# sauloal/pykmer

Measured on AMD Instinct MI355X. Metric: bp/s k-mer counted (k=15, 1 GPU), higher is better.
Workload: dtype u8; 1 GPU; k=15 canonical k-mer count of one 800 Mbp synthetic genome per GPU (SURVEY 8d C2, seed 2+rank), 4^15 table resident in HBM; fasta_bytes=813333854, num_kmers=766212116, parallelism=1 independent genome(s)

## Files before the change

include/pykmer_hip.h:

```cpp
#ifndef PYKMER_HIP_H
#define PYKMER_HIP_H

#include <stddef.h>
#include <stdint.h>

#ifdef __cplusplus
extern "C" {
#endif

#define PK_ABI_VERSION 3

enum {
    PK_OK = 0,
    PK_ERR_ARG = -1,
    PK_ERR_HIP = -2,
    PK_ERR_RECS_CAP = -3,
    PK_ERR_STATE = -4,
    PK_ERR_FORMAT = -5
};

#define PK_FORMAT_FASTA 0
#define PK_FORMAT_FASTQ 1

typedef struct pk_record {
// ... 122 lines not shown
       PK_CORR_FIELDS = 6 };
typedef struct pk_correct pk_correct;
int pk_correct_create(pk_correct **out, int k, int device);
int pk_correct_set_tables(pk_correct *c, const void *const *dev_tables, int N, int min_count, int max_count);
int pk_correct_set_cover(pk_correct *c, const uint8_t *cover, uint64_t n_bases, int min_qual_byte, int min_windows);
int pk_correct_feed(pk_correct *c, const uint8_t *host_text, uint64_t n_bytes, const uint64_t *starts, uint64_t n_records,
                    uint8_t *host_text_out, uint64_t *out);
int pk_correct_feed_device(pk_correct *c, const void *dev_text, uint64_t n_bytes, const uint64_t *starts, uint64_t n_records,
                           void *dev_text_out, uint64_t *out);
int pk_correct_finish(pk_correct *c, uint64_t totals_out[6]);
int pk_correct_timings(pk_correct *c, double out[2]);
void pk_correct_destroy(pk_correct *c);

typedef struct pk_unitig pk_unitig;
int pk_unitig_create(pk_unitig **out, int k, int device);
int pk_unitig_build(pk_unitig *u, const void *dev_table, int min_count, int max_count, uint64_t min_kmers, uint64_t totals_out[8]);
int pk_unitig_rows(pk_unitig *u, uint64_t *first_addr, uint64_t *n_kmers, uint64_t *depth, uint8_t *circular, uint64_t cap);
int pk_unitig_text(pk_unitig *u, uint8_t *host_out, uint64_t offset, uint64_t n_bytes);
int pk_unitig_timings(pk_unitig *u, double out[4]);
void pk_unitig_destroy(pk_unitig *u);

int pk_bgzf_scan(const uint8_t *src, uint64_t n_bytes, uint64_t cap, uint64_t *c_off_out, uint64_t *c_size_out,
                 uint64_t *isize_out, uint64_t *n_blocks_out);
int pk_bgzf_inflate(const uint8_t *src, uint64_t src_bytes, const uint64_t *c_off, const uint64_t *c_size,
                    const uint64_t *u_off, uint64_t n_blocks, uint8_t *dst, int threads);
int pk_bgzf_deflate(const uint8_t *src, uint64_t n_bytes, int level, uint32_t block_input, uint8_t *dst, uint64_t dst_cap,
                    uint64_t *c_sizes_out, uint64_t *total_out, int threads);

int pk_diag_occupancy(int which);
int pk_diag_plan(int k, uint64_t n_bytes, uint64_t out[8]);
int pk_diag_settled_chunks(pk_indexer *ix, uint64_t *out);
int pk_diag_plan_slice(int k, int n_slices, uint64_t n_bytes, uint64_t out[16]);
int pk_diag_level2_order(const uint32_t *sizes, uint32_t B1, uint32_t *order_out);

#ifdef __cplusplus
}
#endif
#endif
```

pykmer_amd/_lib.py:

```python
import ctypes
import os

import numpy as np

_HERE = os.path.dirname(os.path.abspath(__file__))
from ._rt import LIB_PATH, open_library

PK_OK, PK_ERR_ARG, PK_ERR_HIP, PK_ERR_RECS_CAP, PK_ERR_STATE, PK_ERR_FORMAT = 0, -1, -2, -3, -4, -5
PK_FORMAT_FASTA, PK_FORMAT_FASTQ = 0, 1
FORMATS = {"fasta": PK_FORMAT_FASTA, "fastq": PK_FORMAT_FASTQ}
MASK_HARD, MASK_INVERT = 1, 2

RECORD_DTYPE = np.dtype([("name_off", "<u8"), ("name_len", "<u8"), ("seq_len", "<u8"), ("n_valid_kmers", "<u8")])

_u64p = ctypes.POINTER(ctypes.c_uint64)
_SIGNATURES = {
    "pk_version": (ctypes.c_int, []),
    "pk_last_error": (ctypes.c_int, [ctypes.c_char_p, ctypes.c_size_t]),
    "pk_device_count": (ctypes.c_int, []),
    "pk_warm": (ctypes.c_int, [ctypes.c_int]),
    "pk_dev_alloc": (ctypes.c_int, [ctypes.POINTER(ctypes.c_void_p), ctypes.c_uint64, ctypes.c_int]),
    "pk_dev_free": (ctypes.c_int, [ctypes.c_void_p, ctypes.c_int]),
    "pk_dev_upload": (ctypes.c_int, [ctypes.c_void_p, ctypes.c_void_p, ctypes.c_uint64, ctypes.c_int]),
    "pk_dev_download": (ctypes.c_int, [ctypes.c_void_p, ctypes.c_void_p, ctypes.c_uint64, ctypes.c_int]),
# ... 72 lines not shown
    "pk_trim_create": (ctypes.c_int, [ctypes.POINTER(ctypes.c_void_p), ctypes.c_int]),
    "pk_trim_set_cover": (ctypes.c_int, [ctypes.c_void_p, ctypes.c_void_p, ctypes.c_uint64, ctypes.c_int]),
    "pk_trim_feed": (ctypes.c_int, [ctypes.c_void_p, ctypes.c_void_p, ctypes.c_uint64, ctypes.c_void_p, ctypes.c_uint64, ctypes.c_void_p]),
    "pk_trim_feed_device": (ctypes.c_int, [ctypes.c_void_p, ctypes.c_void_p, ctypes.c_uint64, ctypes.c_void_p, ctypes.c_uint64, ctypes.c_void_p]),
    "pk_trim_finish": (ctypes.c_int, [ctypes.c_void_p, ctypes.c_void_p]),
    "pk_trim_timings": (ctypes.c_int, [ctypes.c_void_p, ctypes.c_void_p]),
    "pk_trim_destroy": (None, [ctypes.c_void_p]),
    "pk_correct_create": (ctypes.c_int, [ctypes.POINTER(ctypes.c_void_p), ctypes.c_int, ctypes.c_int]),
    "pk_correct_set_tables": (ctypes.c_int, [ctypes.c_void_p, ctypes.c_void_p, ctypes.c_int, ctypes.c_int, ctypes.c_int]),
    "pk_correct_set_cover": (ctypes.c_int, [ctypes.c_void_p, ctypes.c_void_p, ctypes.c_uint64, ctypes.c_int, ctypes.c_int]),
    "pk_correct_feed": (ctypes.c_int, [ctypes.c_void_p, ctypes.c_void_p, ctypes.c_uint64, ctypes.c_void_p, ctypes.c_uint64, ctypes.c_void_p,
                                        ctypes.c_void_p]),
    "pk_correct_feed_device": (ctypes.c_int, [ctypes.c_void_p, ctypes.c_void_p, ctypes.c_uint64, ctypes.c_void_p, ctypes.c_uint64, ctypes.c_void_p,
                                               ctypes.c_void_p]),
    "pk_correct_finish": (ctypes.c_int, [ctypes.c_void_p, ctypes.c_void_p]),
    "pk_correct_timings": (ctypes.c_int, [ctypes.c_void_p, ctypes.c_void_p]),
    "pk_correct_destroy": (None, [ctypes.c_void_p]),
    "pk_unitig_create": (ctypes.c_int, [ctypes.POINTER(ctypes.c_void_p), ctypes.c_int, ctypes.c_int]),
    "pk_unitig_build": (ctypes.c_int, [ctypes.c_void_p, ctypes.c_void_p, ctypes.c_int, ctypes.c_int, ctypes.c_uint64, ctypes.c_void_p]),
    "pk_unitig_rows": (ctypes.c_int, [ctypes.c_void_p, ctypes.c_void_p, ctypes.c_void_p, ctypes.c_void_p, ctypes.c_void_p, ctypes.c_uint64]),
    "pk_unitig_text": (ctypes.c_int, [ctypes.c_void_p, ctypes.c_void_p, ctypes.c_uint64, ctypes.c_uint64]),
    "pk_unitig_timings": (ctypes.c_int, [ctypes.c_void_p, ctypes.c_void_p]),
    "pk_unitig_destroy": (None, [ctypes.c_void_p]),
    "pk_bgzf_scan": (ctypes.c_int, [ctypes.c_void_p, ctypes.c_uint64, ctypes.c_uint64, ctypes.c_void_p, ctypes.c_void_p, ctypes.c_void_p, _u64p]),
    "pk_bgzf_inflate": (ctypes.c_int, [ctypes.c_void_p, ctypes.c_uint64, ctypes.c_void_p, ctypes.c_void_p, ctypes.c_void_p, ctypes.c_uint64, ctypes.c_void_p,
                                        ctypes.c_int]),
    "pk_bgzf_deflate": (ctypes.c_int, [ctypes.c_void_p, ctypes.c_uint64, ctypes.c_int, ctypes.c_uint32, ctypes.c_void_p, ctypes.c_uint64,
                                        ctypes.c_void_p, _u64p, ctypes.c_int]),
    "pk_diag_occupancy": (ctypes.c_int, [ctypes.c_int]),
    "pk_diag_plan": (ctypes.c_int, [ctypes.c_int, ctypes.c_uint64, ctypes.c_void_p]),
    "pk_diag_settled_chunks": (ctypes.c_int, [ctypes.c_void_p, _u64p]),
    "pk_diag_plan_slice": (ctypes.c_int, [ctypes.c_int, ctypes.c_int, ctypes.c_uint64, ctypes.c_void_p]),
    "pk_diag_level2_order": (ctypes.c_int, [ctypes.c_void_p, ctypes.c_uint32, ctypes.c_void_p]),
}
EXPORTS = tuple(_SIGNATURES)

_lib = None


class PkError(RuntimeError):
    def __init__(self, code, message):
        super().__init__(f"libpykmer_hip error {code}: {message}")
        self.code = code


def load():
    global _lib
    if _lib is None:
        lib = open_library()
        for name, (res, args) in _SIGNATURES.items():
            fn = getattr(lib, name)
            fn.restype, fn.argtypes = res, args
        _lib = lib
    return _lib


def _check(rc):
    if rc != PK_OK:
        buf = ctypes.create_string_buffer(512)
        load().pk_last_error(buf, 512)
        msg = buf.value.decode("utf-8", "replace")
        if rc == PK_ERR_ARG:
            raise ValueError(msg)
        raise PkError(rc, msg)


# ... 689 lines not shown

def bgzf_deflate(data: np.ndarray, level: int, block_input: int, threads: int):
    n_blocks = (data.size + block_input - 1) // block_input
    dst = np.empty(max(1, n_blocks) * 65536, dtype=np.uint8)
    sizes = np.zeros(max(1, n_blocks), dtype=np.uint64)
    total = ctypes.c_uint64(0)
    _check(load().pk_bgzf_deflate(data.ctypes.data, data.size, level, block_input, dst.ctypes.data, dst.size, sizes.ctypes.data,
                                  ctypes.byref(total), int(threads)))
    return dst[: total.value], sizes[:n_blocks].astype(np.int64)


def diag_plan(k: int, n_bytes: int = 0) -> dict:
    out = np.zeros(8, dtype=np.uint64)
    _check(load().pk_diag_plan(k, n_bytes, out.ctypes.data))
    names = ("feed_max", "capacity1", "capacity2", "B1", "B2", "fb_bits", "n_chunks", "fits_u32")
    return {n: int(v) for n, v in zip(names, out)}


WS_VARIANTS = ("narrow", "narrow_sliced", "k15", "k17", "wide_sliced", "deep", "wide")
COUNT_KERNELS = ("whole", "bytes", "half")


def diag_plan_slice(k: int, n_slices: int = 1, n_bytes: int = 0) -> dict:
    out = np.zeros(16, dtype=np.uint64)
    _check(load().pk_diag_plan_slice(k, n_slices, n_bytes, out.ctypes.data))
    names = ("addr_bits", "fb_bits", "b1", "b2", "sample_stride", "n_tally", "sample2", "n_chunks", "variant", "count_kernel",
             "split", "B1", "B2", "capacity1", "capacity2", "fits_u32")
    d = {n: int(v) for n, v in zip(names, out)}
    d["variant"] = WS_VARIANTS[d["variant"]]
    d["count_kernel"] = COUNT_KERNELS[d["count_kernel"]]
    return d


def diag_level2_order(sizes) -> np.ndarray:
    s = np.ascontiguousarray(sizes, dtype=np.uint32)
    out = np.zeros(max(1, s.size), dtype=np.uint32)
    _check(load().pk_diag_level2_order(s.ctypes.data, s.size, out.ctypes.data))
    return out[:s.size]


def gram_expand(pair: np.ndarray) -> np.ndarray:
    p = np.ascontiguousarray(pair, dtype=np.uint64)
    N = p.shape[0]
    m = np.zeros((N, N, 3), dtype=np.uint64)
    _check(load().pk_gram_expand(p.ctypes.data, N, m.ctypes.data))
    return m
```

pykmer_amd/csrc/kmer_part.hip:

```cpp
#include <cstddef>
#include <string>
#include <type_traits>
#include "../../include/pykmer_hip.h"
#include "part_common.h"

namespace pk {

int set_error(int code, const std::string &msg);

__global__ __launch_bounds__(1024) void k_sample2(const uint32_t *__restrict__ in, const uint32_t *__restrict__ bucket_base,
                                                  const uint32_t *__restrict__ bucket_end, PartPlan pl, uint32_t stride2,
                                                  uint32_t *__restrict__ tally, uint32_t *__restrict__ sampled_n,
                                                  const uint32_t *__restrict__ flags) {
    __shared__ uint32_t h[512];
    __shared__ uint32_t n_seen;
    if (flags[0]) return;
    const uint32_t b = blockIdx.x, lo = bucket_base[b], hi = bucket_end[b];
    if (threadIdx.x < 512) h[threadIdx.x] = 0;
    if (threadIdx.x == 0) n_seen = 0;
    __syncthreads();
    const uint32_t n_grp = (hi - lo + 255u) / 256u, n_sgrp = (n_grp + stride2 - 1u) / stride2;
    const uint32_t mask = pl.B2 - 1u, shift = pl.fb_bits, w = threadIdx.x >> 6, lane = threadIdx.x & 63u;
    uint32_t mine = 0;
    for (uint32_t s0 = 0; s0 < n_sgrp; s0 += 8u * 16u) {
// ... 138 lines not shown
            }
            const bool full = v_lo == win && n_tile == (uint32_t)TILE;
            uint32_t okm = 0;
            if (!full) {
#pragma unroll
                for (int j = 0; j < PER / 4; j++) {
                    const uint32_t i = win + (threadIdx.x + j * NT) * 4u;
#pragma unroll
                    for (int e = 0; e < 4; e++) okm |= (i + e >= v_lo && i + e < v_hi) ? (1u << (j * 4 + e)) : 0u;
                }
            }
            if (win + TILE < hi) fetch(win + TILE, nxt);
            uint32_t *cl = cursor + (uint64_t)b * B;
            const uint32_t *ce = cap_end + (uint64_t)b * B;
            if (full) scatter_tile<uint32_t, false, NT, PER, 512, true, 8, REC24>(L, r, 0u, n_tile, shift, B, low_mask, true, out, settle, cl, ce, dump, flags);
            else scatter_tile<uint32_t, false, NT, PER, 512, false, 8, REC24>(L, r, okm, n_tile, shift, B, low_mask, true, out, settle, cl, ce, dump, flags);
        }
    };
    const uint32_t *pos = wg2_start;
    const uint32_t per = pl.B1 >> 3;
    const uint32_t o_lo = (blockIdx.x & 7u) * per, o_hi = o_lo + per, first = blockIdx.x >> 3, step = gridDim.x >> 3;
    const uint32_t w_end = pos[o_hi];
    for (uint32_t w = pos[o_lo] + first; w < w_end; w += step) {
        uint32_t a = o_lo, z = o_hi;
        while (z - a > 1) { const uint32_t m = (a + z) >> 1; if (pos[m] <= w) a = m; else z = m; }
        const uint32_t b = l2_order[a];
        const uint64_t s = (uint64_t)bucket_base[b] + (uint64_t)(w - pos[a]) * pl.R2;
        const uint64_t e = min(s + pl.R2, (uint64_t)bucket_end[b]);
        item(b, (uint32_t)s, (uint32_t)e);
    }
}

constexpr uint32_t K6_PIECE = 65024;
constexpr int K6_BYTES_LDS = 65536 + 1024 + 128;

__device__ __forceinline__ int wave_sum_i32(int v) {
    v += __builtin_amdgcn_update_dpp(0, v, 0x128, 0xf, 0xf, false);
    v += __builtin_amdgcn_update_dpp(0, v, 0x124, 0xf, 0xf, false);
    v += __builtin_amdgcn_update_dpp(0, v, 0x122, 0xf, 0xf, false);
    v += __builtin_amdgcn_update_dpp(0, v, 0x121, 0xf, 0xf, false);
    return __builtin_amdgcn_readlane(v, 0) + __builtin_amdgcn_readlane(v, 16) + __builtin_amdgcn_readlane(v, 32) +
           __builtin_amdgcn_readlane(v, 48);
}

typedef unsigned short U16x2 __attribute__((ext_vector_type(2)));
__device__ __forceinline__ uint32_t clamp255_pair(uint32_t x) {
    const U16x2 lim = {255, 255};
    return __builtin_bit_cast(uint32_t, __builtin_elementwise_min(__builtin_bit_cast(U16x2, x), lim));
}
__device__ __forceinline__ uint32_t pack_low_bytes(uint32_t x0, uint32_t x1) {
    return __builtin_amdgcn_perm(x1, x0, 0x06040200u);
}

struct SliceTally {
    int d1 = 0, d2 = 0;
    __device__ __forceinline__ void add_dword(int *dh, uint32_t x, int sign) {
        uint32_t p0 = x & 0x01010101u, p1 = (x >> 1) & 0x01010101u;
        uint32_t rest = p0 & p1;
        const uint32_t high = x & 0xfcfcfcfcu;
        if (high) {
            const uint32_t big = (((high & 0x7f7f7f7fu) + 0x7f7f7f7fu) | high) & 0x80808080u;
            const uint32_t keep = ~(big >> 7);
            p0 &= keep; p1 &= keep;
            rest = (p0 & p1) | (big >> 7);
        }
        const int n1 = (int)__builtin_popcount(p0 & ~p1), n2 = (int)__builtin_popcount(p1 & ~p0);
        d1 += sign * n1; d2 += sign * n2;
        while (rest) {
            const int bit = __ffs(rest) - 1;
            atomicAdd(&dh[(x >> bit) & 0xffu], sign);
            rest &= rest - 1u;
        }
    }
};

template <int T, bool LEAN, bool NOREC = false>
__device__ __forceinline__ void bucket_count_body(const uint16_t *__restrict__ recs, const uint32_t *__restrict__ final_start,
                                                  const uint32_t *__restrict__ final_end, uint32_t fb_bits, uint32_t split_bits,
                                                  uint8_t *__restrict__ table8, uint32_t fresh, unsigned long long *__restrict__ hist_rep, uint8_t *smem,
                                                  int *dh, uint32_t wg) {
    uint32_t *cnt = reinterpret_cast<uint32_t *>(smem);
    const uint32_t fb = wg >> split_bits, part = wg & ((1u << split_bits) - 1u);
    const uint32_t start = final_start[fb], end = final_end ? final_end[fb] : final_start[fb + 1];
    const uint32_t part_bits = fb_bits - split_bits;
    const uint32_t n_addr = 1u << part_bits;
    uint8_t *slice = table8 + ((uint64_t)fb << fb_bits) + (uint64_t)part * n_addr;
    if (start == end) {
        if (fresh) {
            if (n_addr >= 16) for (uint32_t g = threadIdx.x; g < n_addr / 16; g += T) reinterpret_cast<uint4 *>(slice)[g] = make_uint4(0, 0, 0, 0);
            else for (uint32_t a = threadIdx.x; a < n_addr; a += T) slice[a] = 0;
        }
        return;
    }
    const uint32_t base = start & ~7u;
    const uint32_t i_first = base + threadIdx.x * 8;
    uint4 v_first = make_uint4(0, 0, 0, 0);
    if (i_first < min(base + K6_PIECE, end)) v_first = *reinterpret_cast<const uint4 *>(recs + i_first);
    const bool by_rec = NOREC ? false : (((end - start) >> split_bits) < n_addr / 4 || n_addr < 16);
    SliceTally tally;
    for (uint32_t i = threadIdx.x; i < 256; i += T) dh[i] = 0;
    if (fresh) {
        if (n_addr >= 8) for (uint32_t g = threadIdx.x; g < n_addr / 8; g += T) reinterpret_cast<uint4 *>(cnt)[g] = make_uint4(0, 0, 0, 0);
        else for (uint32_t a = threadIdx.x; a < max(n_addr / 2, 1u); a += T) cnt[a] = 0u;
    } else if (n_addr >= 16) {
        if (!by_rec) __syncthreads();
        for (uint32_t g = threadIdx.x; g < n_addr / 16; g += T) {
            uint4 v = reinterpret_cast<const uint4 *>(slice)[g];
            uint32_t w[4] = {v.x, v.y, v.z, v.w};
            if (!by_rec) {
#pragma unroll
                for (int q = 0; q < 4; q++) tally.add_dword(dh, w[q], -1);
            }
#pragma unroll
            for (int q = 0; q < 8; q++)
                cnt[g * 8 + q] = __builtin_amdgcn_perm(0u, w[q >> 1], (q & 1) ? 0x0c030c02u : 0x0c010c00u);
        }
    } else {
        for (uint32_t a = threadIdx.x; a < max(n_addr / 2, 1u); a += T) cnt[a] = slice[2 * a] | (n_addr > 1u ? (uint32_t)slice[2 * a + 1] << 16 : 0u);
    }
    __syncthreads();
    auto bump = [&](uint32_t a, uint32_t n) {
        const uint32_t sh = 16u * (a & 1u);
        if (!by_rec) { atomicAdd(&cnt[a >> 1], n << sh); return; }
        int &d1 = tally.d1, &d2 = tally.d2;
        const uint32_t c = (atomicAdd(&cnt[a >> 1], n << sh) >> sh) & 0xffffu;
        const uint32_t oc = c > 255u ? 255u : c, nc = c + n > 255u ? 255u : c + n;
        if (oc == nc) return;
        if (nc == 1u) d1++;
        else if (nc == 2u && oc == 1u) { d2++; d1--; }
        else {
            atomicAdd(&dh[nc], 1);
// ... 91 lines not shown
                for (int q = 0; q < 4; q++) tally.add_dword(dh, o[q], 1);
            }
            reinterpret_cast<uint4 *>(slice)[g] = make_uint4(o[0], o[1], o[2], o[3]);
        }
    } else {
        for (uint32_t a = threadIdx.x; a < max(n_addr / 2, 1u); a += T) {
            uint32_t x = cnt[a], lo = x & 0xffffu, hi = x >> 16;
            slice[2 * a] = (uint8_t)(lo > 255u ? 255u : lo);
            if (n_addr > 1u) slice[2 * a + 1] = (uint8_t)(hi > 255u ? 255u : hi);
        }
    }
    const int d1 = wave_sum_i32(tally.d1), d2 = wave_sum_i32(tally.d2);
    if ((threadIdx.x & 63) == 0) {
        if (d1) atomicAdd(&dh[1], d1);
        if (d2) atomicAdd(&dh[2], d2);
    }
    __syncthreads();
    for (uint32_t i = threadIdx.x; i < 256; i += T) {
        const int v = dh[i];
        if (v) atomicAdd(&hist_rep[(uint64_t)(blockIdx.x % HIST_REPLICAS) * 256 + i], (unsigned long long)(long long)v);
    }
}

template <int T>
__global__ __launch_bounds__(T) void k_bucket_count(const uint16_t *__restrict__ recs, const uint32_t *__restrict__ final_start,
                                                    const uint32_t *__restrict__ final_end, uint32_t fb_bits, uint32_t split_bits,
                                                    uint8_t *__restrict__ table8, uint32_t fresh, unsigned long long *__restrict__ hist_rep,
                                                    const uint32_t *__restrict__ flags) {
    extern __shared__ __attribute__((aligned(16))) uint8_t smem[];
    __shared__ int dh[256];
    if (flags[0]) return;
    bucket_count_body<T, true>(recs, final_start, final_end, fb_bits, split_bits, table8, fresh, hist_rep, smem, dh, blockIdx.x);
}
template <int T, bool FRESH>
__global__ __launch_bounds__(T) __attribute__((amdgpu_waves_per_eu(8, 8)))
void k_bucket_count_half_lean(const uint16_t *__restrict__ recs, const uint32_t *__restrict__ final_start, const uint32_t *__restrict__ final_end,
                              uint32_t fb_bits, uint32_t split_bits, uint8_t *__restrict__ table8, uint32_t fresh, unsigned long long *__restrict__ hist_rep,
                              const uint32_t *__restrict__ flags) {
    extern __shared__ __attribute__((aligned(16))) uint8_t smem[];
    __shared__ int dh[256];
    if (flags[0]) return;
    bucket_count_body<T, true, true>(recs, final_start, final_end, 15u, 0u, table8, FRESH ? 1u : 0u, hist_rep, smem, dh, blockIdx.x);
}

template <int T>
__global__ __launch_bounds__(T) __attribute__((amdgpu_waves_per_eu(8, 8)))
void k_bucket_count_bytes(const uint16_t *__restrict__ recs, const uint32_t *__restrict__ final_start, const uint32_t *__restrict__ final_end,
                          uint8_t *__restrict__ table8, uint32_t fresh, unsigned long long *__restrict__ hist_rep,
                          const uint32_t *__restrict__ flags) {
    extern __shared__ __attribute__((aligned(128))) uint8_t smem[];
    constexpr uint32_t N_ADDR = 65536u;
    int *dh = reinterpret_cast<int *>(smem + N_ADDR);
    uint32_t *wrap_flag = reinterpret_cast<uint32_t *>(smem + N_ADDR + 1024);
    if (flags[0]) return;
    const uint32_t fb = blockIdx.x;
    const uint32_t start = final_start[fb], end = final_end ? final_end[fb] : final_start[fb + 1];
    uint4 *slice = reinterpret_cast<uint4 *>(table8 + ((uint64_t)fb << 16));
    uint4 *img = reinterpret_cast<uint4 *>(smem);
    if (start == end) {
        if (fresh) for (uint32_t g = threadIdx.x; g < N_ADDR / 16; g += T) slice[g] = make_uint4(0, 0, 0, 0);
        return;
    }
    bool recount = end - start >= 16384u;
    int d1 = 0, d2 = 0;
    if (!recount) {
        const uint32_t base = start & ~7u;
        const uint32_t i_first = base + threadIdx.x * 8;
        uint4 v = make_uint4(0, 0, 0, 0);
        if (i_first < end) v = *reinterpret_cast<const uint4 *>(recs + i_first);
        for (uint32_t i = threadIdx.x; i < 256; i += T) dh[i] = 0;
        if (threadIdx.x == 0) *wrap_flag = 0u;
        if (fresh) { for (uint32_t g = threadIdx.x; g < N_ADDR / 16; g += T) img[g] = make_uint4(0, 0, 0, 0); }
        else { for (uint32_t g = threadIdx.x; g < N_ADDR / 16; g += T) img[g] = slice[g]; }
        __syncthreads();
        uint32_t *cnt = reinterpret_cast<uint32_t *>(smem);
// ... 145 lines not shown
    pl.n_wg1 = pl.n_chunks < wg1 ? pl.n_chunks : wg1;
    if (pl.n_wg1 == 0) pl.n_wg1 = 1;
    pl.G1 = (pl.n_chunks + pl.n_wg1 - 1) / pl.n_wg1;
    if (pl.G1 == 0) pl.G1 = 1;
    pl.R2 = 4u * TILE;
    pl.sample_stride = pl.n_chunks >= 1024u ? 16u : 1u;
    const uint64_t nfb = (uint64_t)pl.B1 * pl.B2;
    pl.n_tally = (pl.b2 && nfb <= 32768 && pl.addr_bits <= 30) ? (uint32_t)nfb : pl.B1;
    pl.sample2 = (pl.b2 && pl.n_tally == pl.B1 && nfb <= 262144 && pl.B1 >= 8u) ? 1u : 0u;
    const uint64_t est1 = (uint64_t)pl.n_chunks * TILE + pl.B1, est2 = (uint64_t)pl.n_chunks * TILE + nfb;
    pl.capacity1 = est1 + est1 / 8 + (uint64_t)pl.B1 * 4100;
    pl.capacity2 = pl.sample2 ? est2 + est2 / 4 + nfb * 4104 : est2 + est2 / 8 + nfb * 2056;
    return pl;
}

uint32_t bucket_split(const PartPlan &pl, uint64_t n_bytes) {
    return pl.fb_bits == 16 && n_bytes / ((uint64_t)pl.B1 * pl.B2) < 8192u ? 1u : 0u;
}
CountKernel bucket_count_kernel(const PartPlan &pl, uint64_t n_bytes) {
    if (pl.fb_bits == 15) return COUNT_HALF;
    return bucket_split(pl, n_bytes) ? COUNT_BYTES : COUNT_WHOLE;
}

int part_plan_check(const PartPlan &pl, uint64_t n_bytes) {
    const auto no = [](const std::string &what) { return set_error(PK_ERR_HIP, "partition plan outside the kernels' limits: " + what); };
    const uint32_t max_B1 = pl.k <= 15 ? 128u : PART_MAX_B1;
    if (pl.B1 > max_B1 || pl.B2 > 512u || pl.fb_bits > 16u)
        return no(std::to_string(pl.B1) + " x " + std::to_string(pl.B2) + " buckets of 2^" + std::to_string(pl.fb_bits) + " addresses; the LDS arrays hold " +
                  std::to_string(max_B1) + " x 512 of 2^16");
    if (pl.b2 && pl.n_tally == pl.B1 && !pl.sample2) return no("two levels, but neither the sampling launch nor sample2 lays out the final buckets");
    if (pl.k <= 15 && pl.b2 && pl.addr_bits - pl.b1 > 24u)
        return no(std::to_string(pl.addr_bits - pl.b1) + " address bits behind the level-1 digit; its 3-byte records hold 24");
    if (bucket_split(pl, n_bytes) > 1u) return no("the bucket count is laid out for whole and half buckets");
    return PK_OK;
}

size_t part_workspace(const PartPlan &pl, uint64_t n_bytes, uint8_t *base, PartBuffers *view, PartSignals *signals) {
    PartBuffers unused, &b = view ? *view : unused;
    const size_t nfb = (size_t)pl.B1 * pl.B2, rec1 = (size_t)(pl.capacity1 + TILE + 64);
    size_t o = 0;
    const auto place = [&](auto *&p, size_t bytes, bool packed = false) {
        p = reinterpret_cast<std::remove_reference_t<decltype(p)>>(reinterpret_cast<uintptr_t>(base) + o);
        o += bytes;
        if (!packed) o = (o + 255) & ~(size_t)255;
    };
    place(b.codes, (size_t)pl.n_chunks * SLOT_CODE_WORDS * 4);
    place(b.restarts, (size_t)pl.n_chunks * SLOT_RST_WORDS * 4);
    place(b.n_bases, (size_t)pl.n_chunks * 4);
    place(b.tally_rows, (size_t)COUNT_WGS * pl.n_tally * 4);
    const bool s2 = pl.sample2 != 0;
    place(b.tally_tot, (s2 ? nfb : pl.n_tally) * 4, s2);
    place(b.sampled_n, s2 ? (size_t)pl.B1 * 4 : 0, true);
    place(b.block_tot, s2 ? 1024 * 4 : 0);
    if (!s2) b.sampled_n = b.block_tot = nullptr;
    for (uint32_t **p : {&b.bucket_base, &b.bucket_end, &b.cursor1, &b.cap_end, &b.wg2_start}) place(*p, (size_t)(pl.B1 + 1) * 4);
    place(b.l2_order, (size_t)pl.B1 * 4);
    for (uint32_t **p : {&b.final_start, &b.cursor2, &b.cap2_end}) place(*p, (nfb + 1) * 4);
    place(b.out1, !pl.b2 ? rec1 * 2 : pl.k <= 15 ? level1_hi_plane_offset(pl.capacity1) + rec1 : rec1 * 4);
    place(b.out2, !pl.b2 ? 256 : (size_t)(pl.capacity2 + TILE + 64) * 2);
    b.side_cap = n_bytes + 16;
    place(b.side, (size_t)b.side_cap * 8);
    b.signals = signals;
    b.side_n = &b.signals->side_n;
    b.flags = b.signals->flags;
    return o;
}

void part_set_attributes() {
    fuse_set_attributes();
    hipFuncSetAttribute((const void *)k_scatter2<512, 32>, hipFuncAttributeMaxDynamicSharedMemorySize, (int)SCATTER_LDS_NARROW);
    hipFuncSetAttribute((const void *)k_scatter2<512, 32, true>, hipFuncAttributeMaxDynamicSharedMemorySize, (int)SCATTER_LDS_NARROW);
    hipFuncSetAttribute((const void *)k_bucket_count<1024>, hipFuncAttributeMaxDynamicSharedMemorySize, 128 * 1024);
    hipFuncSetAttribute((const void *)k_bucket_count_half_lean<1024, true>, hipFuncAttributeMaxDynamicSharedMemorySize, 128 * 1024);
    hipFuncSetAttribute((const void *)k_bucket_count_half_lean<1024, false>, hipFuncAttributeMaxDynamicSharedMemorySize, 128 * 1024);
    hipFuncSetAttribute((const void *)k_bucket_count_bytes<1024>, hipFuncAttributeMaxDynamicSharedMemorySize, K6_BYTES_LDS);
}

extern "C" int pk_diag_occupancy(int which) {
    int n = -1;
    hipError_t e = hipErrorInvalidValue;
    if (which == 0) e = hipOccupancyMaxActiveBlocksPerMultiprocessor(&n, (const void *)k_bucket_count<1024>, 1024, 128 * 1024);
    if (which == 1) e = hipOccupancyMaxActiveBlocksPerMultiprocessor(&n, (const void *)k_bucket_count_bytes<1024>, 1024, K6_BYTES_LDS);
    if (which == 2) e = hipOccupancyMaxActiveBlocksPerMultiprocessor(&n, (const void *)k_bucket_count_half_lean<1024, true>, 1024, 65536);
    if (which == 3) e = hipOccupancyMaxActiveBlocksPerMultiprocessor(&n, (const void *)k_scatter2<512, 32>, 512, SCATTER_LDS_NARROW);
    return e == hipSuccess ? n : -(int)e;
}

extern "C" int pk_diag_level2_order(const uint32_t *sizes, uint32_t B1, uint32_t *order_out) {
    if (!sizes || !order_out) return set_error(PK_ERR_ARG, "pk_diag_level2_order: null argument");
    static_assert(PART_MAX_B1 == 512, "the message below and include/pykmer_hip.h name the limit");
    if (B1 < 8u || B1 > PART_MAX_B1 || (B1 & 7u)) return set_error(PK_ERR_ARG, "pk_diag_level2_order: B1 must be a multiple of 8 from 8 to 512");
    for (uint32_t b = 0; b < B1; b++) order_out[level2_position(level2_rank(sizes, B1, b), B1)] = b;
    return PK_OK;
}

int launch_partitioned(const PartPlan &pl, const PartBuffers &b, const L2 *st2, uint64_t n_bytes, uint32_t stride, const Carry *carry, uint8_t *table8,
                       unsigned long long *hist, unsigned long long *hist_rep, bool fresh, const PartEvents &ev, hipStream_t s) {
    const uint32_t nfb = pl.B1 * pl.B2;
    const uint32_t *flags = b.flags;
    const char *failed = nullptr;
    hipError_t why = hipSuccess;
    const auto stage = [&](const char *name) { if (!failed && (why = hipGetLastError()) != hipSuccess) failed = name; };
    launch_provision(pl, b, st2, stride, carry, s);
    stage("bucket layout");
    hipEventRecord(ev.sort_begin, s);
    launch_walk_sort(pl, b, st2, carry, s);
    stage("level-1 sort");
    hipEventRecord(ev.sort_end, s);
    const uint16_t *final_recs = (const uint16_t *)b.out1;
    const uint32_t *k6_start = b.bucket_base, *k6_end = b.bucket_end;
    if (pl.sample2) {
        const uint32_t stride2 = stride == 1u ? 1u : 16u, n_blocks = (nfb + 1023u) / 1024u;
        const uint32_t *base1 = b.bucket_base, *end1 = b.bucket_end;
        hipLaunchKernelGGL(k_sample2, dim3(pl.B1), dim3(1024), 0, s, (const uint32_t *)b.out1, base1, end1, pl, stride2, b.tally_tot, b.sampled_n, flags);
        hipLaunchKernelGGL(k_rooms2, dim3(n_blocks), dim3(1024), 0, s, (const uint32_t *)b.tally_tot, (const uint32_t *)b.sampled_n, base1, end1, pl, stride2,
                           nfb, b.final_start, b.cap2_end, b.block_tot, flags);
        hipLaunchKernelGGL(k_bases2, dim3(1), dim3(1024), 0, s, n_blocks, nfb, pl, b.block_tot, b.final_start, b.flags);
        hipLaunchKernelGGL(k_starts2, dim3(n_blocks), dim3(1024), 0, s, nfb, (const uint32_t *)b.block_tot, b.final_start, b.cursor2, b.cap2_end, flags);
        stage("final-bucket rooms");
    }
    if (pl.b2) {
        const uint32_t grid2 = 4096u;
        hipLaunchKernelGGL((pl.k <= 15 ? &k_scatter2<512, 32, true> : &k_scatter2<512, 32>), dim3(grid2), dim3(512), SCATTER_LDS_NARROW, s,
                           (const uint32_t *)b.out1, b.wg2_start, (const uint32_t *)b.l2_order, b.bucket_base, b.bucket_end, pl, b.out2, b.cursor2, (const uint32_t *)b.cap2_end,
                           (uint32_t)pl.capacity2, b.flags);
        stage("level 2");
        final_recs = (const uint16_t *)b.out2; k6_start = b.final_start; k6_end = b.cursor2;
    }
    hipEventRecord(ev.part_end, s);
    const uint32_t split = bucket_split(pl, n_bytes);
    const size_t part_addrs = (size_t)1 << (pl.fb_bits - split);
    const size_t lds6 = part_addrs * 2 < 64 ? 64 : part_addrs * 2;
    const uint32_t n_rows6 = (uint32_t)(nfb << split);
    const auto count = [&](auto kernel, uint32_t grid, size_t lds, auto... geometry) {
        hipLaunchKernelGGL(kernel, dim3(grid), dim3(1024), lds, s, final_recs, k6_start, k6_end, geometry..., table8, fresh ? 1u : 0u, hist_rep, flags);
    };
    switch (bucket_count_kernel(pl, n_bytes)) {
    case COUNT_HALF:
        if (fresh) count(k_bucket_count_half_lean<1024, true>, n_rows6, lds6, pl.fb_bits, split);
        else count(k_bucket_count_half_lean<1024, false>, n_rows6, lds6, pl.fb_bits, split);
        break;
    case COUNT_BYTES: count(k_bucket_count_bytes<1024>, nfb, K6_BYTES_LDS); break;
    case COUNT_WHOLE: count(k_bucket_count<1024>, n_rows6, lds6, pl.fb_bits, split); break;
    }
    stage("bucket count");
    hipLaunchKernelGGL(k_apply_side, dim3(AS_WGS), dim3(WG), 0, s, b.side, b.side_n, b.side_cap, table8, hist, hist_rep, flags);
    stage("side list");
    return failed ? set_error(PK_ERR_HIP, std::string("partition pipeline: the launch of the ") + failed + " failed: " + hipGetErrorString(why)) : PK_OK;
}

}
```

pykmer_amd/csrc/pk_indexer.hip:

```cpp
#include "pk_host.h"

using namespace pk;

static int check_k(int k, int slice_bits = 0, int slice_index = 0) {
    if (k <= 0 || (k % 2) == 0) return fail(PK_ERR_ARG, "kmer_len must be positive and odd (tools.py:165-167), got %d", k);
    if (k > 21) return fail(PK_ERR_ARG, "kmer_len %d not supported by the device path (max 21)", k);
    if (slice_bits < 0 || slice_bits > 2 * k || slice_bits > 16) return fail(PK_ERR_ARG, "bad number of address slices for kmer_len %d", k);
    if (2 * k - slice_bits > 34)
        return fail(PK_ERR_ARG, "kmer_len %d needs a table of 4^%d bytes; one indexer holds 2^34 (16 GiB): count it in %d address slices "
                                "(pk_indexer_create_slice)", k, k, 1 << (2 * k - 34));
    if (slice_index < 0 || slice_index >= (1 << slice_bits)) return fail(PK_ERR_ARG, "slice index %d outside 0..%d", slice_index, (1 << slice_bits) - 1);
    return PK_OK;
}

static int check_slices(int k, int n_slices, int slice_index, int *slice_bits_out) {
    int slice_bits = 0;
    while (slice_bits < 30 && (1 << slice_bits) < n_slices) slice_bits++;
    if (n_slices < 1 || (1 << slice_bits) != n_slices) return fail(PK_ERR_ARG, "the number of address slices must be a power of two, got %d", n_slices);
    *slice_bits_out = slice_bits;
    return check_k(k, slice_bits, slice_index);
}

static int ix_reset(pk_indexer *ix) {
    HIPCHK(hipSetDevice(ix->device));
// ... 128 lines not shown
    if (!out) return fail(PK_ERR_ARG, "null output");
    int rc = check_k(k, k > 17 ? 2 * k - 34 : 0, 0);
    if (rc) return rc;
    if (n_bytes == 0) n_bytes = feed_max_for(k);
    const PartPlan pl = make_part_plan((uint32_t)k, n_bytes, k > 17 ? (uint32_t)(2 * k - 34) : 0u, 0u);
    out[0] = feed_max_for(k); out[1] = pl.capacity1; out[2] = pl.capacity2; out[3] = pl.B1; out[4] = pl.B2; out[5] = pl.fb_bits;
    out[6] = pl.n_chunks; out[7] = plan_fits_u32(pl) ? 1 : 0;
    return PK_OK;
}

extern "C" int pk_diag_settled_chunks(pk_indexer *ix, uint64_t *out) {
    if (!ix || !out) return fail(PK_ERR_ARG, "null argument");
    *out = 0;
    if (!ix->fix_chunks) return PK_OK;
    HIPCHK(hipSetDevice(ix->device));
    std::vector<ChunkFix> fix(ix->fix_chunks);
    HIPCHK(hipMemcpy(fix.data(), ix->chunk_fix.p, fix.size() * sizeof(ChunkFix), hipMemcpyDeviceToHost));
    for (const ChunkFix &f : fix) *out += f.n_lead != 0u;
    return PK_OK;
}

extern "C" int pk_diag_plan_slice(int k, int n_slices, uint64_t n_bytes, uint64_t out[16]) {
    if (!out) return fail(PK_ERR_ARG, "null output");
    int slice_bits = 0;
    int rc = check_slices(k, n_slices, 0, &slice_bits);
    if (rc) return rc;
    if (n_bytes == 0) n_bytes = feed_max_for(k);
    const PartPlan pl = make_part_plan((uint32_t)k, n_bytes, (uint32_t)slice_bits, 0u);
    out[0] = pl.addr_bits; out[1] = pl.fb_bits; out[2] = pl.b1; out[3] = pl.b2; out[4] = pl.sample_stride; out[5] = pl.n_tally;
    out[6] = pl.sample2; out[7] = pl.n_chunks; out[8] = walk_sort_variant(pl); out[9] = bucket_count_kernel(pl, n_bytes);
    out[10] = bucket_split(pl, n_bytes); out[11] = pl.B1; out[12] = pl.B2; out[13] = pl.capacity1; out[14] = pl.capacity2;
    out[15] = plan_fits_u32(pl) ? 1 : 0;
    return PK_OK;
}

template <class Queue>
static int run_feed(pk_indexer *ix, const uint8_t *f, uint64_t n_bytes, const PartPlan &pl, const PartBuffers &pb, const char *what, const char *done,
                    Queue queue) {
    const uint32_t n_chunks = pl.n_chunks;
    int rc = ensure_chunks(ix, n_chunks);
    if (rc) return rc;
    Carry *carry = &ix->tail.p->carry;
    const Events &ev = ix->ev;
    ChunkFix *fix = ix->q ? nullptr : ix->chunk_fix.p;
    ix->fix_chunks = 0;
    HIPCHK(hipEventRecord(ev.scan_begin, ix->stream));
    launch_chunk_l1(f, n_bytes, ix->c_l1.p, n_chunks, ix->stream);
    launch_scan_l1(ix->c_l1.p, n_chunks, carry, ix->c_l1s.p, ix->t_l1.p, pb.signals, ix->stream);
    launch_chunk_l2(f, n_bytes, ix->c_l1s.p, ix->c_l2.p, ix->lane_state.p, ix->packs.p, ix->chunk_odd.p, fix, pb, n_chunks, (uint32_t)ix->k, ix->stream);
    launch_scan_l2(ix->c_l2.p, n_chunks, carry, ix->c_l2s.p, ix->t_l2.p, (uint32_t)ix->k, ix->stream);
    HIPCHK(hipEventRecord(ev.scan_end, ix->stream));
    hipEvent_t squeeze_from = ev.scan_end;
    uint32_t raised = 0;
    uint64_t squeezed_cap = 0;
    for (int attempt = 0;; attempt++) {
        if (attempt) HIPCHK(hipMemsetAsync(pb.signals, 0, sizeof(PartSignals), ix->stream));
        if (!raised || raised == 2u) {
            squeezed_cap = ix->recs_cap();
            if (attempt) { HIPCHK(hipEventRecord(ev.squeeze_begin, ix->stream)); squeeze_from = ev.squeeze_begin; }
            launch_squeeze(pl, pb, f, n_bytes, ix->bytes_fed, ix->lane_state.p, ix->packs.p, ix->c_l2s.p, ix->chunk_odd.p, fix, ix->recs.p, squeezed_cap,
                           carry, ix->stream);
            if (ix->k > 17) launch_deep_tail(pl, pb, carry, ix->stream);
            HIPCHK(hipEventRecord(ev.squeeze_end, ix->stream));
        }
        if ((rc = queue(raised))) return rc;
        if ((rc = read_tail(ix))) return rc;
// ... 501 lines not shown
```

Baseline: 226.6 billion bp/s.

## Replace half-bucket lean count kernel with dense 16-bit LDS counter kernel

Swaps the half-bucket count kernel for a dedicated dense kernel. Each 2^15-address final bucket keeps 16-bit counters in 64 KiB of LDS, incremented with relaxed workgroup-scope LDS atomics, and the byte histogram is maintained with popcount-based tallies instead of per-address walks. The aim is to cut LDS footprint and per-record branching and to raise occupancy, at the cost of a new alignment requirement that is now rejected in the plan check. A diagnostic plan-check entry point is also added.

```diff
diff --git a/include/pykmer_hip.h b/include/pykmer_hip.h
--- a/include/pykmer_hip.h
+++ b/include/pykmer_hip.h
@@ -178,6 +178,7 @@
 int pk_diag_settled_chunks(pk_indexer *ix, uint64_t *out);
 int pk_diag_plan_slice(int k, int n_slices, uint64_t n_bytes, uint64_t out[16]);
 int pk_diag_level2_order(const uint32_t *sizes, uint32_t B1, uint32_t *order_out);
+int pk_diag_plan_check(int k, int n_slices, uint64_t n_bytes, uint32_t fb_bits, uint32_t b1, uint32_t b2);
 
 #ifdef __cplusplus
 }
diff --git a/pykmer_amd/_lib.py b/pykmer_amd/_lib.py
--- a/pykmer_amd/_lib.py
+++ b/pykmer_amd/_lib.py
@@ -128,6 +128,7 @@
     "pk_diag_settled_chunks": (ctypes.c_int, [ctypes.c_void_p, _u64p]),
     "pk_diag_plan_slice": (ctypes.c_int, [ctypes.c_int, ctypes.c_int, ctypes.c_uint64, ctypes.c_void_p]),
     "pk_diag_level2_order": (ctypes.c_int, [ctypes.c_void_p, ctypes.c_uint32, ctypes.c_void_p]),
+    "pk_diag_plan_check": (ctypes.c_int, [ctypes.c_int, ctypes.c_int, ctypes.c_uint64, ctypes.c_uint32, ctypes.c_uint32, ctypes.c_uint32]),
 }
 EXPORTS = tuple(_SIGNATURES)
 
@@ -883,6 +884,10 @@
     return d
 
 
+def diag_plan_check(k: int, n_slices: int, n_bytes: int, fb_bits: int, b1: int, b2: int) -> None:
+    _check(load().pk_diag_plan_check(k, n_slices, n_bytes, fb_bits, b1, b2))
+
+
 def diag_level2_order(sizes) -> np.ndarray:
     s = np.ascontiguousarray(sizes, dtype=np.uint32)
     out = np.zeros(max(1, s.size), dtype=np.uint32)
diff --git a/pykmer_amd/csrc/kmer_part.hip b/pykmer_amd/csrc/kmer_part.hip
--- a/pykmer_amd/csrc/kmer_part.hip
+++ b/pykmer_amd/csrc/kmer_part.hip
@@ -194,6 +194,7 @@
 }
 
 constexpr uint32_t K6_PIECE = 65024;
+constexpr int K6_DENSE_LDS = 65536 + 1024;
 constexpr int K6_BYTES_LDS = 65536 + 1024 + 128;
 
 __device__ __forceinline__ int wave_sum_i32(int v) {
@@ -236,7 +237,7 @@
     }
 };
 
-template <int T, bool LEAN, bool NOREC = false>
+template <int T, bool LEAN>
 __device__ __forceinline__ void bucket_count_body(const uint16_t *__restrict__ recs, const uint32_t *__restrict__ final_start,
                                                   const uint32_t *__restrict__ final_end, uint32_t fb_bits, uint32_t split_bits,
                                                   uint8_t *__restrict__ table8, uint32_t fresh, unsigned long long *__restrict__ hist_rep, uint8_t *smem,
@@ -258,7 +259,7 @@
     const uint32_t i_first = base + threadIdx.x * 8;
     uint4 v_first = make_uint4(0, 0, 0, 0);
     if (i_first < min(base + K6_PIECE, end)) v_first = *reinterpret_cast<const uint4 *>(recs + i_first);
-    const bool by_rec = NOREC ? false : (((end - start) >> split_bits) < n_addr / 4 || n_addr < 16);
+    const bool by_rec = ((end - start) >> split_bits) < n_addr / 4 || n_addr < 16;
     SliceTally tally;
     for (uint32_t i = threadIdx.x; i < 256; i += T) dh[i] = 0;
     if (fresh) {
@@ -416,15 +417,146 @@
     if (flags[0]) return;
     bucket_count_body<T, true>(recs, final_start, final_end, fb_bits, split_bits, table8, fresh, hist_rep, smem, dh, blockIdx.x);
 }
-template <int T, bool FRESH>
-__global__ __launch_bounds__(T) __attribute__((amdgpu_waves_per_eu(8, 8)))
-void k_bucket_count_half_lean(const uint16_t *__restrict__ recs, const uint32_t *__restrict__ final_start, const uint32_t *__restrict__ final_end,
-                              uint32_t fb_bits, uint32_t split_bits, uint8_t *__restrict__ table8, uint32_t fresh, unsigned long long *__restrict__ hist_rep,
-                              const uint32_t *__restrict__ flags) {
-    extern __shared__ __attribute__((aligned(16))) uint8_t smem[];
-    __shared__ int dh[256];
+
+struct DenseTally {
+    uint32_t a = 0, b = 0, c = 0;
+    uint32_t acc[2] = {0, 0};
+    __device__ __forceinline__ void add_dword(uint32_t x, int j) {
+        const uint32_t b1 = x & 0x02020202u;
+        a += (uint32_t)__builtin_popcount(x & 0x01010101u);
+        b += (uint32_t)__builtin_popcount(b1);
+        c += (uint32_t)__builtin_popcount((x << 1) & b1);
+        const uint32_t t = ((x >> 2) & 0x3f3f3f3fu) + 0x3f3f3f3fu;
+        acc[j] = (acc[j] >> 1) | (t & 0x40404040u);
+    }
+    __device__ __forceinline__ void walk(const uint8_t *smem, int *dh, int sign) {
+        uint32_t mask = (acc[0] >> 3) | (acc[1] << 1);
+        const uint32_t own = threadIdx.x * 32u;
+        while (mask) {
+            const uint32_t m = (uint32_t)__builtin_ctz(mask);
+            mask &= mask - 1u;
+            const uint32_t off = own + ((m & 4u) << 13) + ((m & 3u) << 3) + ((m >> 3) << 1);
+            const uint32_t v = min((uint32_t)*reinterpret_cast<const uint16_t *>(smem + off), 255u);
+            atomicAdd(&dh[v], sign);
+            a -= v & 1u; b -= (v >> 1) & 1u; c -= v & (v >> 1) & 1u;
+        }
+    }
+    __device__ __forceinline__ void settle(int sign, int &d1, int &d2, int &d3) {
+        d1 += sign * (int)(a - c); d2 += sign * (int)(b - c); d3 += sign * (int)c;
+        a = b = c = 0; acc[0] = acc[1] = 0;
+    }
+};
+
+template <bool FRESH>
+__global__ __launch_bounds__(1024) __attribute__((amdgpu_waves_per_eu(8, 8)))
+void k_bucket_count_dense(const uint16_t *__restrict__ recs, const uint32_t *__restrict__ final_start, const uint32_t *__restrict__ final_end,
+                          uint32_t, uint32_t, uint8_t *__restrict__ table8, uint32_t, unsigned long long *__restrict__ hist_rep,
+                          const uint32_t *__restrict__ flags) {
+    extern __shared__ __attribute__((aligned(128))) uint8_t smem[];
+    int *dh = reinterpret_cast<int *>(smem + K6_DENSE_LDS - 1024);
+    constexpr uint32_t T = 1024;
+    uint4 *cnt4 = reinterpret_cast<uint4 *>(smem);
+    const uint32_t fb = blockIdx.x, tid = threadIdx.x;
     if (flags[0]) return;
-    bucket_count_body<T, true, true>(recs, final_start, final_end, 15u, 0u, table8, FRESH ? 1u : 0u, hist_rep, smem, dh, blockIdx.x);
+    const uint32_t start = final_start[fb], end = final_end ? final_end[fb] : final_start[fb + 1];
+    uint4 *slice = reinterpret_cast<uint4 *>(table8 + ((uint64_t)fb << 15));
+    if (start == end) {
+        if (FRESH) { slice[tid] = make_uint4(0, 0, 0, 0); slice[tid + T] = make_uint4(0, 0, 0, 0); }
+        return;
+    }
+    const uint32_t i_first = start + tid * 8u;
+    constexpr int NIT = (K6_PIECE + T * 8 - 1) / (T * 8);
+    uint4 v[NIT];
+    if (i_first < min(start + K6_PIECE, end)) v[0] = *reinterpret_cast<const uint4 *>(recs + i_first);
+    if (tid < 256u) dh[tid] = 0;
+    DenseTally tally;
+    int d1 = 0, d2 = 0, d3 = 0;
+    if (FRESH) {
+#pragma unroll
+        for (uint32_t j = 0; j < 4; j++) cnt4[tid + j * T] = make_uint4(0, 0, 0, 0);
+    } else {
+        const uint4 old[2] = {slice[tid], slice[tid + T]};
+        __syncthreads();
+#pragma unroll
+        for (int j = 0; j < 2; j++) {
+            const uint32_t w[4] = {old[j].x, old[j].y, old[j].z, old[j].w};
+            uint32_t c[8];
+#pragma unroll
+            for (int q = 0; q < 4; q++) tally.add_dword(w[q], j);
+#pragma unroll
+            for (int q = 0; q < 8; q++) c[q] = __builtin_amdgcn_perm(0u, w[q >> 1], (q & 1) ? 0x0c030c02u : 0x0c010c00u);
+            cnt4[(tid + j * T) * 2u] = make_uint4(c[0], c[1], c[2], c[3]);
+            cnt4[(tid + j * T) * 2u + 1u] = make_uint4(c[4], c[5], c[6], c[7]);
+        }
+        asm volatile("" ::: "memory");
+        tally.walk(smem, dh, -1);
+        tally.settle(-1, d1, d2, d3);
+    }
+    __syncthreads();
+    typedef __attribute__((address_space(3))) uint32_t lds_u32;
+    const uint32_t ffff = 0xffffu;
+    const auto add = [&](uint32_t x, int odd, bool keep) {
+        const uint32_t off = odd ? ((x >> 15) & 0xfffcu) : ((x << 1) & 0xfffcu);
+        const uint32_t low = odd ? ((x >> 16) & 1u) : (x & 1u);
+        uint32_t val;
+        asm("v_mad_u32_u24 %0, %1, %2, 1" : "=v"(val) : "v"(low), "s"(ffff));
+        if (!keep) val = 0u;
+        __hip_atomic_fetch_add(reinterpret_cast<lds_u32 *>(off), val, __ATOMIC_RELAXED, __HIP_MEMORY_SCOPE_WORKGROUP);
+    };
+    for (uint32_t p0 = start; p0 < end; p0 += K6_PIECE) {
+        const uint32_t p1 = min(p0 + K6_PIECE, end);
+#pragma unroll
+        for (int it = 0; it < NIT; it++) {
+            const uint32_t i = p0 + (tid + it * T) * 8u;
+            if ((it > 0 || p0 != start) && i < p1) v[it] = *reinterpret_cast<const uint4 *>(recs + i);
+        }
+#pragma unroll
+        for (int it = 0; it < NIT; it++) {
+            const uint32_t i = p0 + (tid + it * T) * 8u;
+            const uint32_t w[4] = {v[it].x, v[it].y, v[it].z, v[it].w};
+            if (i + 8u <= p1) {
+#pragma unroll
+                for (int q = 0; q < 8; q++) add(w[q >> 1], q & 1, true);
+            } else if (i < p1) {
+                const uint32_t n = p1 - i;
+#pragma unroll
+                for (int q = 0; q < 8; q++) add(w[q >> 1], q & 1, (uint32_t)q < n);
+            }
+        }
+        __builtin_amdgcn_s_waitcnt(0x0F70);
+        __syncthreads();
+        if (p1 < end) {
+#pragma unroll
+            for (uint32_t j = 0; j < 4; j++) {
+                const uint4 x = cnt4[tid + j * T];
+                cnt4[tid + j * T] = make_uint4(clamp255_pair(x.x), clamp255_pair(x.y), clamp255_pair(x.z), clamp255_pair(x.w));
+            }
+            __syncthreads();
+        }
+    }
+#pragma unroll
+    for (int j = 0; j < 2; j++) {
+        const uint32_t g = tid + j * T;
+        const uint4 c0 = cnt4[g * 2u], c1 = cnt4[g * 2u + 1u];
+        const uint32_t o[4] = {pack_low_bytes(clamp255_pair(c0.x), clamp255_pair(c0.y)), pack_low_bytes(clamp255_pair(c0.z), clamp255_pair(c0.w)),
+                               pack_low_bytes(clamp255_pair(c1.x), clamp255_pair(c1.y)), pack_low_bytes(clamp255_pair(c1.z), clamp255_pair(c1.w))};
+#pragma unroll
+        for (int q = 0; q < 4; q++) tally.add_dword(o[q], j);
+        slice[g] = make_uint4(o[0], o[1], o[2], o[3]);
+    }
+    tally.walk(smem, dh, 1);
+    tally.settle(1, d1, d2, d3);
+    d1 = wave_sum_i32(d1); d2 = wave_sum_i32(d2); d3 = wave_sum_i32(d3);
+    if ((tid & 63u) == 0u) {
+        if (d1) atomicAdd(&dh[1], d1);
+        if (d2) atomicAdd(&dh[2], d2);
+        if (d3) atomicAdd(&dh[3], d3);
+    }
+    __syncthreads();
+    if (tid < 256u) {
+        const int x = dh[tid];
+        if (x) atomicAdd(&hist_rep[(uint64_t)(blockIdx.x % HIST_REPLICAS) * 256 + tid], (unsigned long long)(long long)x);
+    }
 }
 
 template <int T>
@@ -636,6 +768,8 @@
     if (pl.k <= 15 && pl.b2 && pl.addr_bits - pl.b1 > 24u)
         return no(std::to_string(pl.addr_bits - pl.b1) + " address bits behind the level-1 digit; its 3-byte records hold 24");
     if (bucket_split(pl, n_bytes) > 1u) return no("the bucket count is laid out for whole and half buckets");
+    if (pl.fb_bits == 15u && !pl.b2 && pl.B1 > 1u)
+        return no(std::to_string(pl.B1) + " level-1 buckets of 2^15 addresses as final buckets; their starts are multiples of 4 records, the dense count needs 8");
     return PK_OK;
 }
 
@@ -675,8 +809,8 @@
     hipFuncSetAttribute((const void *)k_scatter2<512, 32>, hipFuncAttributeMaxDynamicSharedMemorySize, (int)SCATTER_LDS_NARROW);
     hipFuncSetAttribute((const void *)k_scatter2<512, 32, true>, hipFuncAttributeMaxDynamicSharedMemorySize, (int)SCATTER_LDS_NARROW);
     hipFuncSetAttribute((const void *)k_bucket_count<1024>, hipFuncAttributeMaxDynamicSharedMemorySize, 128 * 1024);
-    hipFuncSetAttribute((const void *)k_bucket_count_half_lean<1024, true>, hipFuncAttributeMaxDynamicSharedMemorySize, 128 * 1024);
-    hipFuncSetAttribute((const void *)k_bucket_count_half_lean<1024, false>, hipFuncAttributeMaxDynamicSharedMemorySize, 128 * 1024);
+    hipFuncSetAttribute((const void *)k_bucket_count_dense<true>, hipFuncAttributeMaxDynamicSharedMemorySize, K6_DENSE_LDS);
+    hipFuncSetAttribute((const void *)k_bucket_count_dense<false>, hipFuncAttributeMaxDynamicSharedMemorySize, K6_DENSE_LDS);
     hipFuncSetAttribute((const void *)k_bucket_count_bytes<1024>, hipFuncAttributeMaxDynamicSharedMemorySize, K6_BYTES_LDS);
 }
 
@@ -685,7 +819,7 @@
     hipError_t e = hipErrorInvalidValue;
     if (which == 0) e = hipOccupancyMaxActiveBlocksPerMultiprocessor(&n, (const void *)k_bucket_count<1024>, 1024, 128 * 1024);
     if (which == 1) e = hipOccupancyMaxActiveBlocksPerMultiprocessor(&n, (const void *)k_bucket_count_bytes<1024>, 1024, K6_BYTES_LDS);
-    if (which == 2) e = hipOccupancyMaxActiveBlocksPerMultiprocessor(&n, (const void *)k_bucket_count_half_lean<1024, true>, 1024, 65536);
+    if (which == 2) e = hipOccupancyMaxActiveBlocksPerMultiprocessor(&n, (const void *)k_bucket_count_dense<true>, 1024, K6_DENSE_LDS);
     if (which == 3) e = hipOccupancyMaxActiveBlocksPerMultiprocessor(&n, (const void *)k_scatter2<512, 32>, 512, SCATTER_LDS_NARROW);
     return e == hipSuccess ? n : -(int)e;
 }
@@ -741,8 +875,8 @@
     };
     switch (bucket_count_kernel(pl, n_bytes)) {
     case COUNT_HALF:
-        if (fresh) count(k_bucket_count_half_lean<1024, true>, n_rows6, lds6, pl.fb_bits, split);
-        else count(k_bucket_count_half_lean<1024, false>, n_rows6, lds6, pl.fb_bits, split);
+        if (fresh) count(k_bucket_count_dense<true>, n_rows6, K6_DENSE_LDS, pl.fb_bits, split);
+        else count(k_bucket_count_dense<false>, n_rows6, K6_DENSE_LDS, pl.fb_bits, split);
         break;
     case COUNT_BYTES: count(k_bucket_count_bytes<1024>, nfb, K6_BYTES_LDS); break;
     case COUNT_WHOLE: count(k_bucket_count<1024>, n_rows6, lds6, pl.fb_bits, split); break;
diff --git a/pykmer_amd/csrc/pk_indexer.hip b/pykmer_amd/csrc/pk_indexer.hip
--- a/pykmer_amd/csrc/pk_indexer.hip
+++ b/pykmer_amd/csrc/pk_indexer.hip
@@ -184,6 +184,20 @@
     out[10] = bucket_split(pl, n_bytes); out[11] = pl.B1; out[12] = pl.B2; out[13] = pl.capacity1; out[14] = pl.capacity2;
     out[15] = plan_fits_u32(pl) ? 1 : 0;
     return PK_OK;
+}
+
+extern "C" int pk_diag_plan_check(int k, int n_slices, uint64_t n_bytes, uint32_t fb_bits, uint32_t b1, uint32_t b2) {
+    int slice_bits = 0;
+    int rc = check_slices(k, n_slices, 0, &slice_bits);
+    if (rc) return rc;
+    if (n_bytes == 0) n_bytes = feed_max_for(k);
+    PartPlan pl = make_part_plan((uint32_t)k, n_bytes, (uint32_t)slice_bits, 0u);
+    if (fb_bits > pl.addr_bits || b1 > 31u || b2 > 31u || fb_bits + b1 + b2 != pl.addr_bits)
+        return fail(PK_ERR_ARG, "pk_diag_plan_check: fb_bits + b1 + b2 must be the plan's %u address bits", pl.addr_bits);
+    const bool tallied = pl.n_tally == pl.B1 * pl.B2;
+    pl.fb_bits = fb_bits; pl.b1 = b1; pl.b2 = b2; pl.B1 = 1u << b1; pl.B2 = 1u << b2;
+    if (tallied) pl.n_tally = pl.B1 * pl.B2;
+    return part_plan_check(pl, n_bytes);
 }
 
 template <class Queue>
```

Result: no change. 228.2 billion bp/s (median of 6 runs) (+0.7%).
